# ljanyst/ssd-tensorflow

Measured on AMD Instinct MI355X. Metric: images/sec (fwd+bwd) vgg300 batch32, higher is better.
Workload: dtype f32; 1 GPU; vgg300 training step (forward + multibox loss + backward + momentum update), 32 images/GPU x 1 GPU, synthetic 300x300 BGR 0..255, GPU-encoded labels, Xavier-init weights (BASELINE.json configs[1]); global_batch=32, parallelism=dp1, allreduce=none

## Files before the change

include/ssdvgg_hip.h:

```cpp
#ifndef SSDVGG_HIP_H
#define SSDVGG_HIP_H

#include <stddef.h>

#ifdef __cplusplus
extern "C" {
#endif

typedef struct ssd_net* ssd_handle;

const char* ssd_last_error(void);
const char* ssd_version(void);

int ssd_preset_info(const char* preset, int* image_w, int* image_h, int* num_anchors, int* num_maps);
int ssd_preset_map(const char* preset, int map, int* size, double* scale, int* num_types);

int ssd_anchors(const char* preset, int device, double* out);
int ssd_anchors_abs(const char* preset, int device, int* out);

int ssd_jaccard_overlap(int device, const double* box, const double* boxes, int n, double* iou_out);

int ssd_encode_labels(const char* preset, int num_classes, int device, const double* gt_boxes,
                      const int* gt_cls, const int* gt_offsets, int b, float* vec_out);
int ssd_encode_labels_dev(const char* preset, int num_classes, int device, const double* gt_boxes,
// ... 360 lines not shown
                               int wi, int ci, int ho, int wo, int co, int kh, int kw, int stride, int dil, int pad_h, int pad_w,
                               void* stream);
int ssd_op_conv2d_dgrad_unpool_bf16(const void* dy, const void* w_io, void* dx_unpooled, const void* rec, int uh, int uw, int b,
                                    int hi, int wi, int ci, int ho, int wo, int co, int kh, int kw, int stride, int dil, int pad_h,
                                    int pad_w, void* stream);
size_t ssd_op_conv2d_dgrad_first_wgrad_bf16_ws_floats(int b, int h, int w);
int ssd_op_conv2d_dgrad_first_wgrad_bf16(const void* dy, const void* w_io, const void* mask, const float* image, float* dw1, float* dbias1,
                                         const float* w1, float weight_decay, float* ws, int b, int h, int w, void* stream);
size_t ssd_op_conv2d_wino_bits_words(int b, int hi, int wi, int ci, int ho, int wo, int co, int kh, int kw, int stride, int dil,
                                     int pad_h, int pad_w);
size_t ssd_op_conv2d_wino_ws_floats(int b, int hi, int wi, int ci, int ho, int wo, int co, int kh, int kw, int stride, int dil,
                                    int pad_h, int pad_w);
int ssd_op_conv2d_wino_fwd(const float* x, const float* w, const float* bias, float* y, float* y_pool, void* rec, void* relu_bits, float* ws,
                           int flags, int b, int hi, int wi, int ci, int ho, int wo, int co, int kh, int kw, int stride, int dil,
                           int pad_h, int pad_w, int relu, void* stream);
int ssd_op_conv2d_wino_dgrad(const float* dy, const float* w, float* dx, const float* mask, const void* mask_bits, int accumulate,
                             const void* rec, int uh, int uw, float* ws, int flags, int b, int hi, int wi, int ci, int ho, int wo, int co,
                             int kh, int kw, int stride, int dil, int pad_h, int pad_w, void* stream);
int ssd_op_conv2d_wino_wgrad(const float* x, const float* dy, float* dw, float* dbias, const float* w, float weight_decay, float* ws,
                             int flags, int b, int hi, int wi, int ci, int ho, int wo, int co, int kh, int kw, int stride, int dil,
                             int pad_h, int pad_w, void* stream);
int ssd_pool_fusion(ssd_handle h, int* out, int cap, int* count);
int ssd_debug_set_ablate(const char* tokens);

int ssd_op_clock_monitor(unsigned* out_dev, int nsamples, unsigned period_ticks, void* stream);
int ssd_op_l2norm_fwd(const float* x, const float* scale, float* y, int npix, int c, void* stream);
size_t ssd_op_l2norm_bwd_ws_floats(int npix, int c);
int ssd_op_l2norm_bwd(const float* x, const float* scale, const float* dy, float* dx, float* dscale,
                      float* ws, int npix, int c, void* stream);

// ... 12 lines not shown
```

ssd_tensorflow_amd/_lib.py:

```python
import ctypes as C
import os

_HERE = os.path.dirname(os.path.abspath(__file__))
LIB_PATH = os.environ.get('SSD_LIB') or os.path.join(_HERE, 'libssdvgg_hip.so')

if not os.path.exists(LIB_PATH):
    raise ImportError(
        f'{LIB_PATH} is missing: build it with `python -c "import __graft_entry__ as g; g.build()"` '
        f'or `make -C {os.path.join(_HERE, "csrc")}` (hipcc, gfx950). There is no CPU fallback.')

try:
    import torch
except ImportError:
    torch = None

lib = C.CDLL(LIB_PATH)

p_f32 = C.POINTER(C.c_float)
p_f64 = C.POINTER(C.c_double)
p_i32 = C.POINTER(C.c_int)
p_i64 = C.POINTER(C.c_longlong)
vp = C.c_void_p
i32 = C.c_int
f32 = C.c_float
# ... 106 lines not shown
    'ssd_merge_tiles_ws_bytes': (sz, [i32, i32]),
    'ssd_merge_tiles_dev': (i32, [vp, i32, i32, i32, vp, vp, vp, vp, vp, i32, i32, i32, vp, vp, vp, vp, vp, vp, vp, vp]),
    'ssd_merge_tiles': (i32, [i32, vp, i32, i32, i32, vp, vp, vp, vp, vp, i32, i32, i32, vp, vp, vp, vp, vp, vp]),
    'ssd_set_overlap': (i32, [handle, i32]),
    'ssd_profile_enable': (i32, [handle, i32]),
    'ssd_profile_report': (i32, [handle, C.c_char_p, sz]),
    'ssd_activation_shape': (i32, [handle, cstr, p_i32, p_i32, p_i32]),
    'ssd_activation': (i32, [handle, cstr, i32, vp, sz]),
    'ssd_op_conv2d_fwd': (i32, [vp, vp, vp, vp] + [i32] * 14 + [vp]),
    'ssd_op_conv2d_dgrad': (i32, [vp, vp, vp, vp, i32] + [i32] * 13 + [vp]),
    'ssd_op_conv2d_wgrad_ws_floats': (sz, [i32] * 13),
    'ssd_op_conv2d_wgrad': (i32, [vp, vp, vp, vp, vp, f32, vp] + [i32] * 13 + [vp]),
    'ssd_op_conv2d_wino_ws_floats': (sz, [i32] * 13),
    'ssd_op_conv2d_wino_bits_words': (sz, [i32] * 13),
    'ssd_op_conv2d_wino_fwd': (i32, [vp, vp, vp, vp, vp, vp, vp, vp, i32] + [i32] * 14 + [vp]),
    'ssd_op_conv2d_wino_dgrad': (i32, [vp, vp, vp, vp, vp, i32, vp, i32, i32, vp, i32] + [i32] * 13 + [vp]),
    'ssd_op_conv2d_wino_wgrad': (i32, [vp, vp, vp, vp, vp, f32, vp, i32] + [i32] * 13 + [vp]),
    'ssd_op_cast_filter': (i32, [vp, vp, vp, i32, i32, i32, vp]),
    'ssd_op_conv2d_fwd_bf16': (i32, [vp, vp, vp, vp, i32] + [i32] * 14 + [vp]),
    'ssd_op_conv2d_dgrad_bf16': (i32, [vp, vp, vp, vp, i32] + [i32] * 13 + [vp]),
    'ssd_op_conv2d_fwd_bf16_chain': (i32, [vp, vp, vp, vp, i32] + [i32] * 14 + [vp]),
    'ssd_op_conv2d_dgrad_bf16_chain': (i32, [vp, vp, vp, vp, i32] + [i32] * 13 + [vp]),
    'ssd_op_conv2d_wgrad_bf16_direct': (i32, [vp, vp, vp, vp, vp, f32] + [i32] * 13 + [vp]),
    'ssd_op_conv2d_wgrad_bf16_ws_floats': (sz, [i32] * 13),
    'ssd_op_conv2d_wgrad_bf16': (i32, [vp, vp, vp, vp, vp, f32, vp] + [i32] * 13 + [vp]),
    'ssd_op_conv2d_first_fwd_bf16': (i32, [vp, vp, vp, vp] + [i32] * 14 + [vp]),
    'ssd_op_conv2d_first_wgrad_bf16_ws_floats': (sz, [i32] * 13),
    'ssd_op_conv2d_first_wgrad_bf16': (i32, [vp, vp, vp, vp, vp, f32, vp] + [i32] * 13 + [vp]),
    'ssd_op_maxpool_rec_fwd': (i32, [vp, vp, vp, i32, i32, i32, i32, i32, vp]),
    'ssd_op_maxpool_rec_bwd': (i32, [vp, vp, vp, i32, i32, i32, i32, i32, i32, vp]),
# ... 74 lines not shown
```

ssd_tensorflow_amd/csrc/api.hip:

```cpp
#include "../../include/ssdvgg_hip.h"
#include "net.h"
#include "augment.h"
#include "annotate.h"
#include "jpeg.h"
#include "jpeg_enc.h"
#include "jpeg_huff.h"
#include "jpeg_huffdec.h"
#include "metrics.h"
#include <vector>
#include <map>
#include <memory>
#include <mutex>
#include <algorithm>

namespace ssd {
static thread_local std::string g_err;
void set_error(const char* fmt, ...) {
    char buf[1024];
    va_list ap;
    va_start(ap, fmt);
    vsnprintf(buf, sizeof buf, fmt, ap);
    va_end(ap);
    g_err = buf;
}
// ... 1253 lines not shown
int ssd_op_conv2d_wino_fwd(const float* x, const float* w, const float* bias, float* y, float* y_pool, void* rec, void* relu_bits, float* ws,
                           int flags, int b, int hi, int wi, int ci, int ho, int wo, int co, int kh, int kw, int stride, int dil,
                           int pad_h, int pad_w, int relu, void* stream) {
    API_BEGIN
    const ConvDesc d = mk(b, hi, wi, ci, ho, wo, co, kh, kw, stride, dil, pad_h, pad_w);
    SSD_REQUIRE(wino_applicable(d), "winograd: 3x3 / stride 1 / SAME layers (any dilation), Ci in multiples of 32, Co of 4");
    const WinoWs k(d, ws);
    if (!(flags & 1)) {
        HIP_OK(hipMemsetAsync(k.Uf, 0, (size_t)36 * d.Ci * wino_kpad(d.Co) * sizeof(float), (hipStream_t)stream));
        wino_filter(d, w, k.U, k.Uf, (hipStream_t)stream);
    }
    wino_fwd(d, x, k.U, bias, y, relu != 0, k.V, (size_t)wino_tiles(d) * d.Ci, k.Mx, y_pool, rec, (hipStream_t)stream, relu_bits,
             (flags & 4) != 0, (flags & 8) != 0);
    API_END
}
int ssd_op_conv2d_wino_dgrad(const float* dy, const float* w, float* dx, const float* mask, const void* mask_bits, int accumulate,
                             const void* rec, int uh, int uw, float* ws, int flags, int b, int hi, int wi, int ci, int ho, int wo, int co,
                             int kh, int kw, int stride, int dil, int pad_h, int pad_w, void* stream) {
    API_BEGIN
    const ConvDesc d = mk(b, hi, wi, ci, ho, wo, co, kh, kw, stride, dil, pad_h, pad_w);
    SSD_REQUIRE(wino_applicable(d), "winograd: 3x3 / stride 1 / SAME layers (any dilation), Ci in multiples of 32, Co of 4");
    const WinoWs k(d, ws);
    if (!(flags & 1)) {
        HIP_OK(hipMemsetAsync(k.Uf, 0, (size_t)36 * d.Ci * wino_kpad(d.Co) * sizeof(float), (hipStream_t)stream));
        wino_filter(d, w, k.U, k.Uf, (hipStream_t)stream);
    }
    wino_bwd_transform(d, dy, k.Yt, nullptr, (hipStream_t)stream, (flags & 8) != 0);
    wino_dgrad(d, k.Yt, k.Uf, dx, mask, accumulate != 0, k.Mx, rec, uh, uw, (hipStream_t)stream, mask_bits, (flags & 4) != 0);
    API_END
}
// ... 296 lines not shown
```

ssd_tensorflow_amd/csrc/conv.h:

```cpp
#pragma once
#include <vector>
#include "common.h"

namespace ssd {

struct ConvDesc {
    int B, Hi, Wi, Ci;
    int Ho, Wo, Co;
    int KH, KW, stride, dil;
    int pad_h, pad_w;
};

void conv_fwd(const ConvDesc& d, const float* x, const float* w, const float* bias,
              float* y, bool relu, hipStream_t s);

void conv_dgrad(const ConvDesc& d, const float* dy, const float* w, float* dx,
                const float* mask, bool accumulate, hipStream_t s);

size_t conv_wgrad_ws_floats(const ConvDesc& d);
void conv_wgrad(const ConvDesc& d, const float* x, const float* dy, float* dw, float* dbias,
                const float* w, float weight_decay, float* ws, hipStream_t s);

bool conv_fwd_pool_supported(const ConvDesc& d);
void conv_fwd_pool(const ConvDesc& d, const float* x, const float* w, const float* bias, float* y_pool, void* rec, hipStream_t s);
// ... 16 lines not shown
    static constexpr int MAX = 24;
    struct Item {
        const float* w;
        float *U, *Uf;
        int Ci, Co, Cop, blk0;
    } it[MAX];
    int n = 0, blocks = 0;
    double elems = 0;
    void add(const float* w, float* U, float* Uf, int Ci, int Co);
};
void wino_filter_plan(const WinoFilterPlan& plan, bool forward, bool flipped, hipStream_t s);
size_t wino_fwd_ws_floats(const ConvDesc& d);
void wino_fwd(const ConvDesc& d, const float* x, const float* U, const float* bias, float* y, bool relu, float* V, size_t v_ps,
              float* Mws, float* y_pool, void* pool_rec, hipStream_t s, void* relu_bits = nullptr, bool two_launch = false,
              bool ref_geom = false);
void wino_bwd_transform(const ConvDesc& d, const float* dy, float* Yt, float* Ya, hipStream_t s, bool ref_geom = false);
size_t wino_dgrad_ws_floats(const ConvDesc& d);
void wino_dgrad(const ConvDesc& d, const float* Yt, const float* Uflip, float* dx, const float* mask, bool accumulate, float* Xws,
                const void* unpool_rec, int UH, int UW, hipStream_t s, const void* mask_bits = nullptr, bool two_launch = false);
size_t wino_wgrad_ws_floats(const ConvDesc& d);
void wino_wgrad(const ConvDesc& d, const float* V, size_t v_ps, const float* Ya, float* dw, float* dbias, const float* w,
                float weight_decay, float* ws, hipStream_t s, bool ref_geom = false);

bool conv_bigk(const ConvDesc& d);
double conv_bigk_useful_flops(const ConvDesc& d);
void conv_bigk_fwd(const ConvDesc& d, const float* x, const float* w, const float* bias, float* y, bool relu, hipStream_t s);
void conv_bigk_dgrad(const ConvDesc& d, const float* dy, const float* w, float* dx, const float* mask, bool accumulate, hipStream_t s);
void conv_bigk_wgrad(const ConvDesc& d, const float* x, const float* dy, float* dw, float* dbias, const float* w, float weight_decay,
                     hipStream_t s);

// ... 128 lines not shown
```

ssd_tensorflow_amd/csrc/net.h:

```cpp
#pragma once
#include "common.h"
#include "conv.h"
#include "ops.h"
#include "boxes.h"
#include "bf16.h"
#include <string>
#include <vector>
#include <map>

namespace ssd {

struct Tensor {
    std::string name;
    int H = 0, W = 0, C = 0;
    bool relu_out = false;
    int consumers = 0;
    int done = 0;
    int gstream = 0;
    long gseq = 0;
    hipEvent_t gev = nullptr;
    bool gev_set = false;
    bool data_f32 = true;
    bool grad_f32 = true;
    void* data = nullptr;
// ... 20 lines not shown
    size_t w_off = 0, b_off = 0;
    size_t ws_off = 0;
    int k = 2;
    void* pool_rec = nullptr;
    bool fused_fwd = false, fused_bwd = false;
    int pool_after = -1, unpool = -1;
    int head = -1;
    bool fp8 = false;
    size_t sw_off = 0;
    size_t w6_off = 0;
    bool wino_f = false, wino_d = false, wino_w = false;
    float *wino_U = nullptr, *wino_Uf = nullptr, *wino_V = nullptr;
    void* wino_bits = nullptr;
    long long wino_bits_step = -1;
    long long wino_v_step = -1;
};

struct Variable {
    std::string name;
    int ndim;
    int shape[4];
    size_t off, rows, width, pitch;
    size_t count() const { return rows * width; }
};

struct DetectSlot {
    char* dev = nullptr;
    char* host = nullptr;
    size_t bytes = 0, used = 0;
    int b = 0, out_cap = 0;
// ... 185 lines not shown
```

ssd_tensorflow_amd/csrc/net.hip:

```cpp
#include "net.h"
#include <cmath>
#include <algorithm>
#include <cstdlib>
#include <atomic>
#include <mutex>

namespace ssd {

static bool first_layer_kernel(const ConvDesc& d) { return d.Ci * d.KH * d.KW <= 32 && d.Co == 64; }

int Net::add_tensor(const std::string& name, int H, int W, int C, bool relu_out) {
    Tensor t;
    t.name = name; t.H = H; t.W = W; t.C = C; t.relu_out = relu_out;
    tensors_.push_back(t);
    return (int)tensors_.size() - 1;
}

enum PadMode { PAD_SAME, PAD_VALID, PAD_BR1_VALID };

void Net::build_graph() {
    const Preset& p = *preset_;
    const int nv = C_ + 5;
    input_t_ = add_tensor("image_input", p.image_h, p.image_w, 3, false);
    int cur = input_t_;
// ... 452 lines not shown
        if (op.wino_d) {
            op.wino_Uf = (float*)hip_.mem(uf * sizeof(float));
            HIP_OK(hipMemset(op.wino_Uf, 0, uf * sizeof(float)));
            yt_max = std::max(yt_max, t * wino_kpad(d.Co));
            xw_max = std::max(xw_max, t * d.Ci);
        }
        if (op.wino_w) {
            yt_max = std::max(yt_max, t * wino_kpad(d.Co));
            for (int b = 1; b <= Bmax_; ++b) slab_max = std::max(slab_max, wino_wgrad_ws_floats(conv_desc(op, b)));
        }
        (wino_plan_first_.n == 0 && op.wino_f ? wino_plan_first_ : wino_plan_).add(params_ + op.w_off, op.wino_U, nullptr, d.Ci, d.Co);
        if (op.wino_Uf) wino_plan_flip_.add(params_ + op.w_off, nullptr, op.wino_Uf, d.Ci, d.Co);
        wino_any_f_ |= op.wino_f;
        wino_any_d_ |= op.wino_d;
    }
    if (wino_plan_.n + wino_plan_first_.n + wino_plan_flip_.n == 0) return;
    ev_wino_ = hip_.event();
    ev_wino_first_ = hip_.event();
    ev_wino_flip_ = hip_.event();
    if (m_max) for (int l = 0; l < 3; ++l) wino_m_[l] = (float*)hip_.mem(m_max * sizeof(float));
    if (v_max) for (int l = 0; l < 3; ++l) wino_vs_[l] = (float*)hip_.mem(v_max * sizeof(float));
    if (training_) {
        wino_yt_ = (float*)hip_.mem(yt_max * sizeof(float));
        wino_xw_ = (float*)hip_.mem(xw_max * sizeof(float));
        wino_ya_ = (float*)hip_.mem(yt_max * sizeof(float));
        wino_slab_ = (float*)hip_.mem(slab_max * sizeof(float));
    }
}

void Net::plan_fp8() {
// ... 403 lines not shown
        bool armed = false;
        bool done = false;
        explicit LossSlotGuard(long long& s) : seq(s) {}
        void failed() { if (armed && !done) { --seq; armed = false; } }
        ~LossSlotGuard() { if (armed && !done) --seq; }
    } fwd_guard(loss_seq_);
    if (train_mode) {
        begin_loss_slot();
        fwd_guard.armed = true;
        prof_.layer = "loss";
        l2_partials(params_, nfilters_, lw_, side ? hstream_ : stream_);
        if (nl == 2) HIP_OK(hipEventRecord(ev_l2_, hstream_));
    }
    int nl_cur = nl;
    int small_heads = 0;
    for (const int op_index : fwd_order_) {
        const Op& op = ops_[op_index];
        const Tensor& in = tensors_[op.in];
        const Tensor& out = tensors_[op.out];
        prof_.layer = op.name.c_str();
        if (op_ablated(op.name, op.kind, op.head, op.k)) continue;
        if (chain_fwd_ && in_chain_[op_index]) {
            if (op_index == chain_first_)
                for (int li = 0; li < nl_cur; ++li) {
                    Lane& ln = lane[li];
                    if (ln.cast_pending) {
                        HIP_OK(hipStreamWaitEvent(ln.s, ev_cast_, 0));
                        ln.cast_pending = false;
                    }
                    launch_tail_forward(ln.b0, ln.nb, ln.s);
                }
            continue;
        }
        if (nl_cur == 2 && heads_full && op_index == tail_first_) {
            HIP_OK(hipEventRecord(ev_join_, s2_));
            HIP_OK(hipStreamWaitEvent(stream_, ev_join_, 0));
            lane[0].nb = b;
            nl_cur = 1;
        }
        for (int li = 0; li < nl_cur; ++li) {
            Lane& ln = lane[li];
            const int nb = ln.nb;
            switch (op.kind) {
            case OP_CONV: {
                hipStream_t cs = ln.s;
                int run_nb = nb, run_b0 = ln.b0;
                if (op.head >= 0 && side) {
                    if (!ln.fmap_carried[op.head]) HIP_OK(hipEventRecord(ln.ev_fmap[op.head], ln.s));
                    ln.fmap_carried[op.head] = false;
                    if (heads_full) {
                        if (li < nl_cur - 1) break;
                        cs = (nl_cur == 1 && op.head >= 2 && (small_heads++ & 1)) ? s2_ : hstream_;
                        for (int l = 0; l < nl_cur; ++l) HIP_OK(hipStreamWaitEvent(cs, lane[l].ev_fmap[op.head], 0));
                        run_nb = b; run_b0 = 0;
                        lane[0].heads_on_side = true;
                    } else {
                        HIP_OK(hipStreamWaitEvent(ln.h, ln.ev_fmap[op.head], 0));
                        cs = ln.h;
                        ln.heads_on_side = true;
// ... 22 lines not shown
                    }
                    const size_t tpi = (size_t)wino_tiles(d) / d.B;
                    if (op.wino_V) {
                        wino_V = op.wino_V + (size_t)run_b0 * tpi * d.Ci;
                        wino_vps = (size_t)b * tpi * d.Ci;
                        if (train_mode) ops_[op_index].wino_v_step = fwd_serial_;
                    } else {
                        wino_V = wino_vs_[cs == ln.s ? li : 2];
                        wino_vps = (size_t)run_nb * tpi * d.Ci;
                    }
                    if (train_mode && op.wino_bits) {
                        wino_bits = static_cast<char*>(op.wino_bits) + (size_t)run_b0 * tpi * (d.Ci / 4) * 8;
                        ops_[op_index].wino_bits_step = fwd_serial_;
                    }
                }
                if (op.pool_after >= 0) {
                    const Op& pl = ops_[op.pool_after];
                    const Tensor& pt = tensors_[pl.out];
                    void* rec = (pl.pool_rec && train_mode)
                                    ? static_cast<char*>(pl.pool_rec) + (size_t)run_b0 * pt.H * pt.W * (pt.C / 4) * sizeof(unsigned short) : nullptr;
                    if (wino)
                        wino_fwd(d, xin, op.wino_U, params_ + op.b_off, nullptr, true, wino_V, wino_vps, wino_M,
                                 reinterpret_cast<float*>(at(pt, run_b0)), rec, cs, wino_bits);
                    else if (!bf16_)
                        conv_fwd_pool(d, xin, params_ + op.w_off, params_ + op.b_off, reinterpret_cast<float*>(at(pt, run_b0)), rec, cs);
                    else
                        conv_fwd_pool_bf16(d, reinterpret_cast<const bf16_t*>(xin), wq_oi_ + op.w_off, params_ + op.b_off,
                                           reinterpret_cast<bf16_t*>(at(pt, run_b0)), rec, cs);
                    if (run8 && pt.data8)
                        quantize8(pt, at(pt, run_b0), run_b0, run_nb, cs);
                    break;
                }
                const int fh = (side && op.head < 0 && cs == ln.s) ? head_of(op.out) : -1;
                if (fh >= 0) g_stop_event = ln.ev_fmap[fh];
                struct CarryScope {
                    bool* flag;
                    ~CarryScope() { if (flag) *flag = g_stop_event == nullptr; g_stop_event = nullptr; }
                } carry_scope{fh >= 0 ? &ln.fmap_carried[fh] : nullptr};
                if (wino)
                    wino_fwd(d, xin, op.wino_U, params_ + op.b_off, static_cast<float*>(yout), op.relu, wino_V, wino_vps, wino_M,
                             nullptr, nullptr, cs, wino_bits);
                else if (!bf16_)
                    conv_fwd(d, xin, params_ + op.w_off, params_ + op.b_off, static_cast<float*>(yout), op.relu, cs);
                else if (in.data_f32 && first_layer_kernel(d))
                    conv_first_fwd_bf16(d, xin, params_ + op.w_off, params_ + op.b_off, static_cast<bf16_t*>(yout), op.relu, cs);
                else if (in.data_f32)
                    conv_fwd_smallc_bf16out(d, xin, params_ + op.w_off, params_ + op.b_off, static_cast<bf16_t*>(yout), op.relu, cs);
                else if (run8 && op.fp8 && mx6_)
                    conv_fwd_mxfp6(d, in.data8 + (size_t)run_b0 * (in.per_image() / 32 * 24), in.scale8 + (size_t)run_b0 * (in.per_image() / 32),
                                   w8_ + op.w6_off, wsc6_ + op.sw_off, params_ + op.b_off, yout,
                                   out.data8 ? out.data8 + (size_t)run_b0 * (out.per_image() / 32 * 24) : nullptr,
                                   out.data8 ? out.scale8 + (size_t)run_b0 * (out.per_image() / 32) : nullptr,
                                   out.data8 ? (out.wants16 ? FP8_OUT_BF16_MX : FP8_OUT_MX) : FP8_OUT_BF16, op.relu, cs);
                else if (run8 && op.fp8 && mx_)
// ... 94 lines not shown
}

void Net::launch_wgrad(int op_index, int b, hipStream_t ws) {
    const Op& op = ops_[op_index];
    const Tensor& in = tensors_[op.in];
    const Tensor& out = tensors_[op.out];
    const ConvDesc d = conv_desc(op, b);
    float* slab = wgrad_ws_ + op.ws_off;
    prof_.layer = op.name.c_str();
    if (op.wino_w && op.wino_v_step == fwd_serial_) {
        const size_t tpi = (size_t)wino_tiles(d) / d.B;
        wino_bwd_transform(d, out.gf(), nullptr, wino_ya_, ws);
        wino_wgrad(d, op.wino_V, (size_t)b * tpi * d.Ci, wino_ya_, grads_ + op.w_off, grads_ + op.b_off, params_ + op.w_off, wd_,
                   wino_slab_, ws);
    } else if (!bf16_) {
        conv_wgrad(d, in.f(), out.gf(), grads_ + op.w_off, grads_ + op.b_off, params_ + op.w_off, wd_, slab, ws);
    } else if (in.data_f32) {
        if (first_layer_kernel(d))
            conv_first_wgrad_bf16(d, in.f(), out.gh(), grads_ + op.w_off, grads_ + op.b_off, params_ + op.w_off, wd_, slab, ws);
        else
            conv_wgrad_smallc_bf16dy(d, in.f(), out.gh(), grads_ + op.w_off, grads_ + op.b_off, params_ + op.w_off, wd_, slab, ws);
    } else {
        conv_wgrad_bf16(d, in.h(), out.gh(), grads_ + op.w_off, grads_ + op.b_off, params_ + op.w_off, wd_, slab, ws);
    }
}

void Net::backward_begin(int b, const float* y) {
    SSD_REQUIRE(training_, "handle was created with training = 0");
    g_prof = &prof_;
    prof_.layer = "loss";
// ... 80 lines not shown
                        if (ops_[j].kind == OP_CONV && ops_[j].out == op.in && ops_[j].in == input_t_) first = j;
                if (first >= 0 && cls == 0 && conv_dgrad_first_wgrad_bf16_applicable(d, conv_desc(ops_[first], b))) {
                    const Op& f = ops_[first];
                    prof_.layer = "conv1_2+conv1_1";
                    conv_dgrad_first_wgrad_bf16(d, out.gh(), wq_io_ + op.w_off, in.h(), conv_desc(f, b), tensors_[input_t_].f(),
                                                grads_ + f.w_off, grads_ + f.b_off, params_ + f.w_off, wd_, wgrad_ws_ + f.ws_off, ds);
                    bw_first_fused_ = true;
                    fused_first_out_ = op.in;
                    bw_wrote(cls, in);
                    bw_conv_done_[op_index] = 1;
                    lo = bw_final_lo();
                    break;
                }
                g_stop_event = dst.gev;
                struct Disarm { ~Disarm() { g_stop_event = nullptr; } } disarm;
                if (op.wino_d && cls == 0) {
                    wino_bwd_transform(d, out.gf(), wino_yt_, nullptr, ds);
                    wino_dgrad(d, wino_yt_, op.wino_Uf, up ? dst.gf() : in.gf(), mask ? in.f() : nullptr, !up && in.done > 0, wino_xw_,
                               up ? up->pool_rec : nullptr, dst.H, dst.W, ds,
                               op.wino_bits && op.wino_bits_step == fwd_serial_ ? op.wino_bits : nullptr);
                } else if (!bf16_) {
                    if (up) conv_dgrad_unpool(d, out.gf(), params_ + op.w_off, dst.gf(), up->pool_rec, dst.H, dst.W, ds);
                    else conv_dgrad(d, out.gf(), params_ + op.w_off, in.gf(), mask ? in.f() : nullptr, in.done > 0, ds);
                } else {
                    if (up) conv_dgrad_unpool_bf16(d, out.gh(), wq_io_ + op.w_off, dst.gh(), up->pool_rec, dst.H, dst.W, ds);
                    else conv_dgrad_bf16(d, out.gh(), wq_io_ + op.w_off, in.gh(), mask ? in.h() : nullptr, in.done > 0, ds);
                }
                const bool carried = dst.gev && g_stop_event == nullptr;
                bw_wrote(cls, dst, carried);
            }
            bw_conv_done_[op_index] = 1;
            lo = bw_final_lo();
            break;
        }
        case OP_POOL: {
// ... 219 lines not shown
    const bool want_bf16 = name && !strncmp(name, "bf16:", 5);
    if (want_bf16) name += 5;
    const bool want_scale = name && !want_grad && !want_bf16 && !strncmp(name, "scale:", 6);
    if (want_scale) name += 6;
    for (size_t ti = 0; ti < tensors_.size(); ++ti) {
        const Tensor& t = tensors_[ti];
        if (t.name != name || !t.data) continue;
        SSD_REQUIRE(!want_grad || t.grad != nullptr, "no gradient storage (training = 0?)");
        SSD_REQUIRE(!(want_grad && bw_first_fused_ && fused_first_out_ == (int)ti),
                    "gradient of %s is not materialised: the first layer's weight gradient was computed inside the next layer's data gradient (SSD_POOL_FUSE=3 keeps it)", name);
        for (const Op& op : ops_) {
            SSD_REQUIRE(!(op.kind == OP_POOL && op.fused_fwd && op.in == (int)ti && !want_grad),
                        "activation %s is not materialised: its 2x2 pool is fused into the convolution (SSD_POOL_FUSE=0 keeps it)", name);
            SSD_REQUIRE(!(op.kind == OP_POOL && op.fused_bwd && op.out == (int)ti && want_grad),
                        "gradient of %s is not materialised: the pool's backward is fused into its consumer's data gradient (SSD_POOL_FUSE=0 keeps it)", name);
        }
        if (want_scale) {
            SSD_REQUIRE(t.scale8 != nullptr, "activation %s has no block scales (not an MX tensor of an mxfp8 handle)", name);
            SSD_REQUIRE(count == t.per_image() / 32 * b, "scale:%s holds %zu floats for b=%d, got %zu", name, t.per_image() / 32 * b, b, count);
            HIP_OK(hipStreamSynchronize(stream_));
            std::vector<unsigned char> hs(count);
            HIP_OK(hipMemcpy(hs.data(), t.scale8, count, hipMemcpyDeviceToHost));
            for (size_t i = 0; i < count; ++i) out[i] = ldexpf(1.f, (int)hs[i] - 127);
            return;
        }
        SSD_REQUIRE(count == t.per_image() * b, "activation %s holds %zu floats for b=%d, got %zu", name, t.per_image() * b, b,
                    count);
        const void* src = want_grad ? t.grad : t.data;
        HIP_OK(hipStreamSynchronize(stream_));
        if (t.data8 && !want_grad && !want_bf16 && mx6_) {
// ... 124 lines not shown
```

ssd_tensorflow_amd/csrc/winograd.hip:

```cpp
#include "conv.h"
#include "conv_detail.h"
#include "bf16.h"
#include <algorithm>
#include <cmath>

namespace ssd {

#define LDS_PTR(p) ((__attribute__((address_space(3))) void*)(p))
constexpr unsigned WOOB = 0xFFFFFFF0u;

__device__ __forceinline__ void bt6(f32x4& d0, f32x4& d1, f32x4& d2, f32x4& d3, f32x4& d4, f32x4& d5) {
    const f32x4 t0 = 1.265625f * d0 - 2.8125f * d2 + d4;
    const f32x4 e = d4 - 2.25f * d2, f = 1.6875f * d1 - 0.75f * d3;
    const f32x4 g = d4 - 0.5625f * d2, h = 0.84375f * d1 - 1.5f * d3;
    const f32x4 t5 = 1.265625f * d1 - 2.8125f * d3 + d5;
    d0 = t0; d1 = e - f; d2 = e + f; d3 = g - h; d4 = g + h; d5 = t5;
}
__device__ __forceinline__ void a6(const f32x4 e0, const f32x4 e1, const f32x4 e2, const f32x4 e3, f32x4* u) {
    const f32x4 p = e0 + 0.5625f * e2, q = 0.75f * e1 + 0.421875f * e3;
    const f32x4 r = e0 + 2.25f * e2, t = 1.5f * e1 + 3.375f * e3;
    u[0] = e0;
    u[1] = p + q;
    u[2] = p - q;
    u[3] = r + t;
    u[4] = r - t;
    u[5] = e3;
}
template <class V>
__device__ __forceinline__ void at4(const V m0, const V m1, const V m2, const V m3, const V m4, const V m5, V* y) {
    const V s12 = m1 + m2, d12 = m1 - m2, s34 = m3 + m4, d34 = m3 - m4;
    y[0] = m0 + s12 + s34;
    y[1] = 0.75f * d12 + 1.5f * d34;
    y[2] = 0.5625f * s12 + 2.25f * s34;
    y[3] = 0.421875f * d12 + 3.375f * d34 + m5;
}

__host__ __device__ inline int bias_axis_slot(int k) { return k == 0 ? 0 : k == 1 ? 1 : k == 2 ? 2 : k == 5 ? 3 : -1; }
__device__ __forceinline__ float bias_axis_weight(int slot) {
    return slot == 0 ? -7.f / 9.f : slot == 1 ? 14.f / 9.f : slot == 2 ? 2.f / 9.f : 7.f / 16.f;
}

template <bool BT, bool AT>
__global__ __launch_bounds__(256) void wino_in_kernel(const float* __restrict__ x, float* __restrict__ V, float* __restrict__ Va,
                                                      int H, int W, int C, int Cp, int th, int tw, int T, unsigned x_bytes,
                                                      size_t v_ps, size_t va_ps, int D, unsigned long long* __restrict__ bits,
                                                      bool raster) {
    const int c4n = Cp >> 2;
    const int wg = (BT && !raster) ? xcd_remap(blockIdx.x, gridDim.x) : (int)blockIdx.x;
    const int idx = wg * 256 + threadIdx.x;
    const int q = idx % c4n, t = idx / c4n;
    if (t >= T) return;
    const int j = t % tw, t2 = t / tw;
    const int i = t2 % th, b = t2 / th;
    const int hb = (i % D) + D * 4 * (i / D), wb = (j % D) + D * 4 * (j / D);
// ... 1 lines not shown
    constexpr int LO = BT ? 0 : 1, HI = BT ? 6 : 5;
    f32x4 d[6][6];
#pragma unroll
    for (int r = LO; r < HI; ++r) {
        const int h = hb + D * (r - 1);
        const bool hv = (unsigned)h < (unsigned)H;
#pragma unroll
        for (int s = LO; s < HI; ++s) {
            const int w = wb + D * (s - 1);
            const bool ok = hv && (unsigned)w < (unsigned)W && q * 4 < C;
            const unsigned off = ok ? (unsigned)(((b * H + h) * W + w) * C + q * 4) * 4u : WOOB;
            d[r][s] = __builtin_bit_cast(f32x4, __builtin_amdgcn_raw_buffer_load_b128(rs, off, 0, 0));
        }
    }
    const size_t row = (size_t)t * Cp + q * 4;
    if constexpr (BT) {
        if (bits) {
            unsigned long long m = 0;
#pragma unroll
            for (int r = 0; r < 4; ++r)
#pragma unroll
                for (int s = 0; s < 4; ++s)
#pragma unroll
                    for (int e = 0; e < 4; ++e) m |= (unsigned long long)(d[r + 1][s + 1][e] > 0.f) << ((r * 4 + s) * 4 + e);
            bits[(size_t)t * c4n + q] = m;
        }
    }
    if constexpr (AT) {
        f32x4 c[6][4];
#pragma unroll
        for (int s = 0; s < 4; ++s) {
            f32x4 u[6];
            a6(d[1][s + 1], d[2][s + 1], d[3][s + 1], d[4][s + 1], u);
#pragma unroll
            for (int k = 0; k < 6; ++k) c[k][s] = u[k];
        }
#pragma unroll
        for (int k = 0; k < 6; ++k) {
            f32x4 u[6];
            a6(c[k][0], c[k][1], c[k][2], c[k][3], u);
#pragma unroll
            for (int l = 0; l < 6; ++l) *reinterpret_cast<f32x4*>(Va + (size_t)(k * 6 + l) * va_ps + row) = u[l];
        }
    }
    if constexpr (BT) {
#pragma unroll
        for (int s = 0; s < 6; ++s) bt6(d[0][s], d[1][s], d[2][s], d[3][s], d[4][s], d[5][s]);
#pragma unroll
        for (int r = 0; r < 6; ++r) {
            bt6(d[r][0], d[r][1], d[r][2], d[r][3], d[r][4], d[r][5]);
#pragma unroll
            for (int s = 0; s < 6; ++s) *reinterpret_cast<f32x4*>(V + (size_t)(r * 6 + s) * v_ps + row) = d[r][s];
        }
    }
}

struct WinoOutArgs {
    const float* M;
    size_t m_ps;
    float* y;
    const float* bias;
    const float* mask;
    const unsigned long long* mask_bits;
    int relu, accum;
    int H, W, N, th, tw, T;
    int D;
    unsigned short* pool_rec;
    int PH, PW;
// ... 790 lines not shown
        auto kern = wino_gemm_out_kernel<MODE, 1>;
        static bool once = (set_lds(kern, lds), true);
        (void)once;
        SSD_LAUNCH_STOP(kern, dim3(cdiv(a.M, 32) * a.NT), dim3(512), lds, s, a);
    } else {
        auto kern = wino_gemm_out_kernel<MODE, 2>;
        static bool once = (set_lds(kern, lds), true);
        (void)once;
        SSD_LAUNCH_STOP(kern, dim3(cdiv(a.M, 32) * a.NT), dim3(512), lds, s, a);
    }
    HIP_OK(hipGetLastError());
}

size_t wino_fwd_ws_floats(const ConvDesc& d) { return (size_t)36 * wino_tiles(d) * d.Co; }

void wino_fwd(const ConvDesc& d, const float* x, const float* U, const float* bias, float* y, bool relu, float* V, size_t v_ps,
              float* Mws, float* y_pool, void* pool_rec, hipStream_t s, void* relu_bits, bool two_launch, bool ref_geom) {
    require(d);
    const int T = wino_tiles(d);
    launch_in(x, V, nullptr, d.B, d.Hi, d.Wi, d.Ci, d.Ci, d.dil, v_ps, 0, s, static_cast<unsigned long long*>(relu_bits), ref_geometry(ref_geom, GEOM_IN));
    const bool fused = fuse_out(d, d.Co, d.Ci, two_launch);
    if (!fused) gemm_nn(V, v_ps, U, Mws, (size_t)T * d.Co, T, d.Co, d.Ci, s);
    WinoOutArgs a{};
    a.M = Mws; a.m_ps = (size_t)T * d.Co; a.bias = bias; a.relu = relu; a.H = d.Ho; a.W = d.Wo; a.N = d.Co;
    a.th = tiles_1d(d.Ho, d.dil); a.tw = tiles_1d(d.Wo, d.dil); a.T = T; a.D = d.dil;
    const double mb = 4.0 * 36 * T * d.Co;
    if (y_pool) {
        SSD_REQUIRE(d.dil == 1, "winograd: the fused pool is for undilated layers");
        a.y = y_pool; a.pool_rec = static_cast<unsigned short*>(pool_rec); a.PH = (d.Ho + 1) / 2; a.PW = (d.Wo + 1) / 2;
        const double ob = 4.0 * d.B * a.PH * a.PW * d.Co;
        if (fused) launch_fused<2>(V, v_ps, U, d.Ci, a, ob, s);
        else launch_out<2>(a, "wino_out_pool", mb + ob, s);
    } else {
        a.y = y;
        const double ob = 4.0 * d.B * d.Ho * d.Wo * d.Co;
// ... 108 lines not shown
```

Baseline: 1437 images/s.

## Fuse first VGG conv into the Winograd input transform of conv1_2

Adds a kernel that computes the first 3x3 conv (3 image channels to 64) with MFMA on a tile of image pixels, applies bias and ReLU, keeps the result in LDS, and writes the Winograd input transform and ReLU mask bits for the second conv directly. The first layer's 64-channel activation at full 300x300 resolution is then never written to or read back from global memory. In exchange, the halo pixels around each tile are recomputed. The weight gradient of the first layer and any activation query must now cope with that tensor being absent, so guards and a recompute path for activation queries are added.

Result: no change. 1447 images/s, median of 5 (+0.8%).

```diff
diff --git a/include/ssdvgg_hip.h b/include/ssdvgg_hip.h
--- a/include/ssdvgg_hip.h
+++ b/include/ssdvgg_hip.h
@@ -398,6 +398,9 @@
 int ssd_op_conv2d_wino_fwd(const float* x, const float* w, const float* bias, float* y, float* y_pool, void* rec, void* relu_bits, float* ws,
                            int flags, int b, int hi, int wi, int ci, int ho, int wo, int co, int kh, int kw, int stride, int dil,
                            int pad_h, int pad_w, int relu, void* stream);
+int ssd_op_conv2d_wino_fwd_first(const float* image, int image_c, const float* w1, const float* bias1, const float* w, const float* bias,
+                                 float* y, float* y_pool, void* rec, void* relu_bits, float* ws, int flags, int b, int hi, int wi, int ci,
+                                 int ho, int wo, int co, int kh, int kw, int stride, int dil, int pad_h, int pad_w, int relu, void* stream);
 int ssd_op_conv2d_wino_dgrad(const float* dy, const float* w, float* dx, const float* mask, const void* mask_bits, int accumulate,
                              const void* rec, int uh, int uw, float* ws, int flags, int b, int hi, int wi, int ci, int ho, int wo, int co,
                              int kh, int kw, int stride, int dil, int pad_h, int pad_w, void* stream);
diff --git a/ssd_tensorflow_amd/_lib.py b/ssd_tensorflow_amd/_lib.py
--- a/ssd_tensorflow_amd/_lib.py
+++ b/ssd_tensorflow_amd/_lib.py
@@ -144,6 +144,7 @@
     'ssd_op_conv2d_wino_ws_floats': (sz, [i32] * 13),
     'ssd_op_conv2d_wino_bits_words': (sz, [i32] * 13),
     'ssd_op_conv2d_wino_fwd': (i32, [vp, vp, vp, vp, vp, vp, vp, vp, i32] + [i32] * 14 + [vp]),
+    'ssd_op_conv2d_wino_fwd_first': (i32, [vp, i32, vp, vp, vp, vp, vp, vp, vp, vp, vp, i32] + [i32] * 14 + [vp]),
     'ssd_op_conv2d_wino_dgrad': (i32, [vp, vp, vp, vp, vp, i32, vp, i32, i32, vp, i32] + [i32] * 13 + [vp]),
     'ssd_op_conv2d_wino_wgrad': (i32, [vp, vp, vp, vp, vp, f32, vp, i32] + [i32] * 13 + [vp]),
     'ssd_op_cast_filter': (i32, [vp, vp, vp, i32, i32, i32, vp]),
diff --git a/ssd_tensorflow_amd/csrc/api.hip b/ssd_tensorflow_amd/csrc/api.hip
--- a/ssd_tensorflow_amd/csrc/api.hip
+++ b/ssd_tensorflow_amd/csrc/api.hip
@@ -1291,6 +1291,23 @@
              (flags & 4) != 0, (flags & 8) != 0);
     API_END
 }
+int ssd_op_conv2d_wino_fwd_first(const float* image, int image_c, const float* w1, const float* bias1, const float* w, const float* bias,
+                                 float* y, float* y_pool, void* rec, void* relu_bits, float* ws, int flags, int b, int hi, int wi, int ci,
+                                 int ho, int wo, int co, int kh, int kw, int stride, int dil, int pad_h, int pad_w, int relu, void* stream) {
+    API_BEGIN
+    const ConvDesc d = mk(b, hi, wi, ci, ho, wo, co, kh, kw, stride, dil, pad_h, pad_w);
+    const ConvDesc d1 = mk(b, hi, wi, image_c, hi, wi, ci, 3, 3, 1, 1, 1, 1);
+    SSD_REQUIRE(wino_fwd_first_applicable(d1, d),
+                "winograd, first-layer form: image channels * 9 <= 32 into 64 channels, then an undilated 3x3 / stride 1 / SAME layer");
+    const WinoWs k(d, ws);
+    if (!(flags & 1)) {
+        HIP_OK(hipMemsetAsync(k.Uf, 0, (size_t)36 * d.Ci * wino_kpad(d.Co) * sizeof(float), (hipStream_t)stream));
+        wino_filter(d, w, k.U, k.Uf, (hipStream_t)stream);
+    }
+    wino_fwd_first(d1, image, w1, bias1, d, k.U, bias, y, relu != 0, k.V, (size_t)wino_tiles(d) * d.Ci, k.Mx, y_pool, rec,
+                   (hipStream_t)stream, relu_bits, (flags & 4) != 0);
+    API_END
+}
 int ssd_op_conv2d_wino_dgrad(const float* dy, const float* w, float* dx, const float* mask, const void* mask_bits, int accumulate,
                              const void* rec, int uh, int uw, float* ws, int flags, int b, int hi, int wi, int ci, int ho, int wo, int co,
                              int kh, int kw, int stride, int dil, int pad_h, int pad_w, void* stream) {
diff --git a/ssd_tensorflow_amd/csrc/conv.h b/ssd_tensorflow_amd/csrc/conv.h
--- a/ssd_tensorflow_amd/csrc/conv.h
+++ b/ssd_tensorflow_amd/csrc/conv.h
@@ -54,6 +54,10 @@
 void wino_fwd(const ConvDesc& d, const float* x, const float* U, const float* bias, float* y, bool relu, float* V, size_t v_ps,
               float* Mws, float* y_pool, void* pool_rec, hipStream_t s, void* relu_bits = nullptr, bool two_launch = false,
               bool ref_geom = false);
+bool wino_fwd_first_applicable(const ConvDesc& d1, const ConvDesc& d);
+void wino_fwd_first(const ConvDesc& d1, const float* image, const float* w1, const float* bias1, const ConvDesc& d, const float* U,
+                    const float* bias, float* y, bool relu, float* V, size_t v_ps, float* Mws, float* y_pool, void* pool_rec, hipStream_t s,
+                    void* relu_bits = nullptr, bool two_launch = false);
 void wino_bwd_transform(const ConvDesc& d, const float* dy, float* Yt, float* Ya, hipStream_t s, bool ref_geom = false);
 size_t wino_dgrad_ws_floats(const ConvDesc& d);
 void wino_dgrad(const ConvDesc& d, const float* Yt, const float* Uflip, float* dx, const float* mask, bool accumulate, float* Xws,
diff --git a/ssd_tensorflow_amd/csrc/net.h b/ssd_tensorflow_amd/csrc/net.h
--- a/ssd_tensorflow_amd/csrc/net.h
+++ b/ssd_tensorflow_amd/csrc/net.h
@@ -58,6 +58,8 @@
     void* wino_bits = nullptr;
     long long wino_bits_step = -1;
     long long wino_v_step = -1;
+    int wino_first_into = -1, wino_first = -1;
+    long long wino_first_step = -1;
 };
 
 struct Variable {
diff --git a/ssd_tensorflow_amd/csrc/net.hip b/ssd_tensorflow_amd/csrc/net.hip
--- a/ssd_tensorflow_amd/csrc/net.hip
+++ b/ssd_tensorflow_amd/csrc/net.hip
@@ -490,6 +490,22 @@
         wino_any_f_ |= op.wino_f;
         wino_any_d_ |= op.wino_d;
     }
+    static const int first_on = env_i("SSD_WINO_FIRST", 1);
+    if (first_on)
+        for (int i = 0; i < (int)ops_.size(); ++i) {
+            Op& f = ops_[i];
+            if (f.kind != OP_CONV || f.in != input_t_ || !f.relu || f.head >= 0 || tensors_[f.out].consumers != 1) continue;
+            for (int j = 0; j < (int)ops_.size(); ++j) {
+                Op& c = ops_[j];
+                if (c.in != f.out) continue;
+                if (c.kind != OP_CONV || !c.wino_f || c.dil != 1 || c.head >= 0) break;
+                if (training_ && !(c.wino_d && c.wino_w && c.wino_bits)) break;
+                if (!wino_fwd_first_applicable(conv_desc(f, Bmax_), conv_desc(c, Bmax_))) break;
+                f.wino_first_into = j;
+                c.wino_first = i;
+                break;
+            }
+        }
     if (wino_plan_.n + wino_plan_first_.n + wino_plan_flip_.n == 0) return;
     ev_wino_ = hip_.event();
     ev_wino_first_ = hip_.event();
@@ -923,6 +939,10 @@
     }
     int nl_cur = nl;
     int small_heads = 0;
+    auto first_fused = [&](int first, int second, int li) {
+        const Op &f = ops_[first], &c = ops_[second];
+        return c.wino_f && wino_m_[li] != nullptr && !op_ablated(f.name, f.kind, f.head, f.k) && !op_ablated(c.name, c.kind, c.head, c.k);
+    };
     for (const int op_index : fwd_order_) {
         const Op& op = ops_[op_index];
         const Tensor& in = tensors_[op.in];
@@ -952,6 +972,7 @@
             const int nb = ln.nb;
             switch (op.kind) {
             case OP_CONV: {
+                if (op.wino_first_into >= 0 && first_fused(op_index, op.wino_first_into, li)) break;
                 hipStream_t cs = ln.s;
                 int run_nb = nb, run_b0 = ln.b0;
                 if (op.head >= 0 && side) {
@@ -1004,12 +1025,19 @@
                         ops_[op_index].wino_bits_step = fwd_serial_;
                     }
                 }
+                const Op* first = (wino && cs == ln.s && op.wino_first >= 0 && first_fused(op.wino_first, op_index, li)) ? &ops_[op.wino_first] : nullptr;
+                const float* image = first ? reinterpret_cast<const float*>(at(tensors_[first->in], run_b0)) : nullptr;
+                if (first) ops_[op_index].wino_first_step = fwd_serial_;
                 if (op.pool_after >= 0) {
                     const Op& pl = ops_[op.pool_after];
                     const Tensor& pt = tensors_[pl.out];
                     void* rec = (pl.pool_rec && train_mode)
                                     ? static_cast<char*>(pl.pool_rec) + (size_t)run_b0 * pt.H * pt.W * (pt.C / 4) * sizeof(unsigned short) : nullptr;
-                    if (wino)
+                    if (first)
+                        wino_fwd_first(conv_desc(*first, run_nb), image, params_ + first->w_off, params_ + first->b_off, d, op.wino_U,
+                                       params_ + op.b_off, nullptr, true, wino_V, wino_vps, wino_M, reinterpret_cast<float*>(at(pt, run_b0)),
+                                       rec, cs, wino_bits);
+                    else if (wino)
                         wino_fwd(d, xin, op.wino_U, params_ + op.b_off, nullptr, true, wino_V, wino_vps, wino_M,
                                  reinterpret_cast<float*>(at(pt, run_b0)), rec, cs, wino_bits);
                     else if (!bf16_)
@@ -1027,7 +1055,11 @@
                     bool* flag;
                     ~CarryScope() { if (flag) *flag = g_stop_event == nullptr; g_stop_event = nullptr; }
                 } carry_scope{fh >= 0 ? &ln.fmap_carried[fh] : nullptr};
-                if (wino)
+                if (first)
+                    wino_fwd_first(conv_desc(*first, run_nb), image, params_ + first->w_off, params_ + first->b_off, d, op.wino_U,
+                                   params_ + op.b_off, static_cast<float*>(yout), op.relu, wino_V, wino_vps, wino_M, nullptr, nullptr, cs,
+                                   wino_bits);
+                else if (wino)
                     wino_fwd(d, xin, op.wino_U, params_ + op.b_off, static_cast<float*>(yout), op.relu, wino_V, wino_vps, wino_M,
                              nullptr, nullptr, cs, wino_bits);
                 else if (!bf16_)
@@ -1152,6 +1184,7 @@
         wino_wgrad(d, op.wino_V, (size_t)b * tpi * d.Ci, wino_ya_, grads_ + op.w_off, grads_ + op.b_off, params_ + op.w_off, wd_,
                    wino_slab_, ws);
     } else if (!bf16_) {
+        SSD_REQUIRE(op.wino_first_step != fwd_serial_, "%s: the weight gradient would read an activation the forward pass did not write", op.name.c_str());
         conv_wgrad(d, in.f(), out.gf(), grads_ + op.w_off, grads_ + op.b_off, params_ + op.w_off, wd_, slab, ws);
     } else if (in.data_f32) {
         if (first_layer_kernel(d))
@@ -1262,11 +1295,14 @@
                 }
                 g_stop_event = dst.gev;
                 struct Disarm { ~Disarm() { g_stop_event = nullptr; } } disarm;
+                const bool bits_ok = op.wino_bits && op.wino_bits_step == fwd_serial_;
+                SSD_REQUIRE(!(mask && op.wino_first_step == fwd_serial_ && !(op.wino_d && cls == 0 && bits_ok)),
+                            "%s: the data gradient's mask would read an activation the forward pass did not write", op.name.c_str());
                 if (op.wino_d && cls == 0) {
                     wino_bwd_transform(d, out.gf(), wino_yt_, nullptr, ds);
                     wino_dgrad(d, wino_yt_, op.wino_Uf, up ? dst.gf() : in.gf(), mask ? in.f() : nullptr, !up && in.done > 0, wino_xw_,
                                up ? up->pool_rec : nullptr, dst.H, dst.W, ds,
-                               op.wino_bits && op.wino_bits_step == fwd_serial_ ? op.wino_bits : nullptr);
+                               bits_ok ? op.wino_bits : nullptr);
                 } else if (!bf16_) {
                     if (up) conv_dgrad_unpool(d, out.gf(), params_ + op.w_off, dst.gf(), up->pool_rec, dst.H, dst.W, ds);
                     else conv_dgrad(d, out.gf(), params_ + op.w_off, in.gf(), mask ? in.f() : nullptr, in.done > 0, ds);
@@ -1516,6 +1552,10 @@
                         "activation %s is not materialised: its 2x2 pool is fused into the convolution (SSD_POOL_FUSE=0 keeps it)", name);
             SSD_REQUIRE(!(op.kind == OP_POOL && op.fused_bwd && op.out == (int)ti && want_grad),
                         "gradient of %s is not materialised: the pool's backward is fused into its consumer's data gradient (SSD_POOL_FUSE=0 keeps it)", name);
+            if (op.kind == OP_CONV && op.out == (int)ti && !want_grad && op.wino_first_into >= 0 &&
+                ops_[op.wino_first_into].wino_first_step == fwd_serial_ && fwd_serial_ > 0)
+                conv_fwd(conv_desc(op, b), tensors_[input_t_].f(), params_ + op.w_off, params_ + op.b_off, static_cast<float*>(t.data), op.relu,
+                         stream_);
         }
         if (want_scale) {
             SSD_REQUIRE(t.scale8 != nullptr, "activation %s has no block scales (not an MX tensor of an mxfp8 handle)", name);
diff --git a/ssd_tensorflow_amd/csrc/winograd.hip b/ssd_tensorflow_amd/csrc/winograd.hip
--- a/ssd_tensorflow_amd/csrc/winograd.hip
+++ b/ssd_tensorflow_amd/csrc/winograd.hip
@@ -38,6 +38,28 @@
 __host__ __device__ inline int bias_axis_slot(int k) { return k == 0 ? 0 : k == 1 ? 1 : k == 2 ? 2 : k == 5 ? 3 : -1; }
 __device__ __forceinline__ float bias_axis_weight(int slot) {
     return slot == 0 ? -7.f / 9.f : slot == 1 ? 14.f / 9.f : slot == 2 ? 2.f / 9.f : 7.f / 16.f;
+}
+
+__device__ __forceinline__ void wino_bt_store(f32x4 (&d)[6][6], float* __restrict__ V, size_t v_ps, size_t row,
+                                              unsigned long long* __restrict__ bits, size_t word) {
+    if (bits) {
+        unsigned long long m = 0;
+#pragma unroll
+        for (int r = 0; r < 4; ++r)
+#pragma unroll
+            for (int s = 0; s < 4; ++s)
+#pragma unroll
+                for (int e = 0; e < 4; ++e) m |= (unsigned long long)(d[r + 1][s + 1][e] > 0.f) << ((r * 4 + s) * 4 + e);
+        bits[word] = m;
+    }
+#pragma unroll
+    for (int s = 0; s < 6; ++s) bt6(d[0][s], d[1][s], d[2][s], d[3][s], d[4][s], d[5][s]);
+#pragma unroll
+    for (int r = 0; r < 6; ++r) {
+        bt6(d[r][0], d[r][1], d[r][2], d[r][3], d[r][4], d[r][5]);
+#pragma unroll
+        for (int s = 0; s < 6; ++s) *reinterpret_cast<f32x4*>(V + (size_t)(r * 6 + s) * v_ps + row) = d[r][s];
+    }
 }
 
 template <bool BT, bool AT>
@@ -69,18 +91,6 @@
         }
     }
     const size_t row = (size_t)t * Cp + q * 4;
-    if constexpr (BT) {
-        if (bits) {
-            unsigned long long m = 0;
-#pragma unroll
-            for (int r = 0; r < 4; ++r)
-#pragma unroll
-                for (int s = 0; s < 4; ++s)
-#pragma unroll
-                    for (int e = 0; e < 4; ++e) m |= (unsigned long long)(d[r + 1][s + 1][e] > 0.f) << ((r * 4 + s) * 4 + e);
-            bits[(size_t)t * c4n + q] = m;
-        }
-    }
     if constexpr (AT) {
         f32x4 c[6][4];
 #pragma unroll
@@ -98,15 +108,130 @@
             for (int l = 0; l < 6; ++l) *reinterpret_cast<f32x4*>(Va + (size_t)(k * 6 + l) * va_ps + row) = u[l];
         }
     }
-    if constexpr (BT) {
-#pragma unroll
-        for (int s = 0; s < 6; ++s) bt6(d[0][s], d[1][s], d[2][s], d[3][s], d[4][s], d[5][s]);
-#pragma unroll
-        for (int r = 0; r < 6; ++r) {
-            bt6(d[r][0], d[r][1], d[r][2], d[r][3], d[r][4], d[r][5]);
-#pragma unroll
-            for (int s = 0; s < 6; ++s) *reinterpret_cast<f32x4*>(V + (size_t)(r * 6 + s) * v_ps + row) = d[r][s];
-        }
+    if constexpr (BT) wino_bt_store(d, V, v_ps, row, bits, (size_t)t * c4n + q);
+}
+
+constexpr int FB_R = 2, FB_C = 4;
+constexpr int FB_PH = 4 * FB_R + 2, FB_PW = 4 * FB_C + 2, FB_PIX = FB_PH * FB_PW;
+constexpr int FB_ROW = 64;
+__device__ __forceinline__ int fb_slot(int px, int c) { return px * FB_ROW + ((c ^ (px & 7)) << 2); }
+constexpr int FB_THREADS = FB_R * FB_C * 16;
+constexpr int FB_KMAX = 28;
+struct WinoFirstArgs {
+    const float* x;
+    const float* w;
+    const float* bias;
+    float* V;
+    unsigned long long* bits;
+    size_t v_ps;
+    int H, W, Ci, ntaps, th, tw, bh, bw, nblk;
+    unsigned x_bytes;
+    int tap_dh[9], tap_dw[9];
+};
+
+__device__ __forceinline__ void fb_lds_barrier() {
+    asm volatile("s_waitcnt lgkmcnt(0)" ::: "memory");
+    __builtin_amdgcn_s_barrier();
+}
+
+__global__ __launch_bounds__(FB_THREADS, 2) void wino_in_first_kernel(WinoFirstArgs p) {
+    __shared__ __attribute__((aligned(16))) float act[FB_PIX * FB_ROW];
+    __shared__ __attribute__((aligned(16))) float sbias[64];
+    __shared__ float sw[FB_KMAX * 64];
+    __shared__ int ktab[2][16][2];
+    const int tid = threadIdx.x, wave = tid >> 6, lane = tid & 63;
+    const int li = lane & 31, lh = lane >> 5;
+    const int K = p.ntaps * p.Ci;
+    for (int e = tid; e < FB_KMAX * 64; e += FB_THREADS) sw[e] = e < K * 64 ? p.w[e] : 0.f;
+    if (tid < 64) sbias[tid] = p.bias ? p.bias[tid] : 0.f;
+    if (tid < 32) {
+        const int k = 2 * (tid & 15) + (tid >> 4);
+        const bool kv = k < K;
+        const int tp = kv ? k / p.Ci : 0, c = kv ? k - tp * p.Ci : 0;
+        ktab[tid >> 4][tid & 15][0] = ((p.tap_dh[tp] * p.W + p.tap_dw[tp]) * p.Ci + c) * 4;
+        ktab[tid >> 4][tid & 15][1] = kv ? (1 << tp) : 0;
+    }
+    __syncthreads();
+    const __amdgpu_buffer_rsrc_t x_rsrc = __builtin_amdgcn_make_buffer_rsrc(const_cast<float*>(p.x), 0, p.x_bytes, 0x00020000);
+    const int tl = tid >> 4, q = tid & 15;
+    const int ty = tl / FB_C, tx = tl - ty * FB_C;
+
+    constexpr int NG = (FB_PIX + 31) / 32, NW = FB_THREADS / 64, FB_GPW = NG / NW;
+    static_assert(NG % NW == 0, "every wave takes the same number of pixel groups");
+    float xb[FB_GPW][16];
+    auto gather = [&](int blk) {
+        const int bj = blk % p.bw, b2 = blk / p.bw;
+        const int bi = b2 % p.bh, b = b2 / p.bh;
+        int lhb = lh;
+        asm volatile("" : "+v"(lhb));
+#pragma unroll
+        for (int gi = 0; gi < FB_GPW; ++gi) {
+            const int px = (wave + NW * gi) * 32 + li;
+            const int ry = px / FB_PW, rx = px - ry * FB_PW;
+            const int h = 4 * FB_R * bi - 1 + ry, w = 4 * FB_C * bj - 1 + rx;
+            const bool inside = px < FB_PIX && (unsigned)h < (unsigned)p.H && (unsigned)w < (unsigned)p.W;
+            unsigned mk = 0;
+            for (int t = 0; t < p.ntaps; ++t) {
+                const int sh = h + p.tap_dh[t], sw = w + p.tap_dw[t];
+                if ((unsigned)sh < (unsigned)p.H && (unsigned)sw < (unsigned)p.W) mk |= 1u << t;
+            }
+            if (!inside) mk = 0;
+            const unsigned base = (unsigned)(((b * p.H + h) * p.W + w) * p.Ci) * 4u;
+#pragma unroll
+            for (int j = 0; j < 16; ++j) {
+                const unsigned ok = 0u - (unsigned)((mk & (unsigned)ktab[lhb][j][1]) != 0u);
+                xb[gi][j] = __builtin_bit_cast(float, __builtin_amdgcn_raw_buffer_load_b32(x_rsrc, (int)(((base + (unsigned)ktab[lhb][j][0]) & ok) | (WOOB & ~ok)), 0, 0));
+            }
+        }
+    };
+
+    for (int blk = blockIdx.x; blk < p.nblk; blk += gridDim.x) {
+        const int bj = blk % p.bw, b2 = blk / p.bw;
+        const int bi = b2 % p.bh, b = b2 / p.bh;
+        gather(blk);
+#pragma unroll
+        for (int gi = 0; gi < FB_GPW; ++gi) {
+            const int px = (wave + NW * gi) * 32 + li;
+            const bool live = px < FB_PIX;
+            const int ry = px / FB_PW, rx = px - ry * FB_PW;
+            const int h = 4 * FB_R * bi - 1 + ry, w = 4 * FB_C * bj - 1 + rx;
+            const bool inside = live && (unsigned)h < (unsigned)p.H && (unsigned)w < (unsigned)p.W;
+#pragma unroll
+            for (int nt = 0; nt < 2; ++nt) {
+                f32x16 acc;
+#pragma unroll
+                for (int r = 0; r < 16; ++r) acc[r] = 0.f;
+#pragma unroll
+                for (int j = 0; j < 16; ++j) acc = __builtin_amdgcn_mfma_f32_32x32x2f32(2 * j + 1 < FB_KMAX ? sw[(2 * j + lh) * 64 + nt * 32 + li] : 0.f, xb[gi][j], acc, 0, 0, 0);
+#pragma unroll
+                for (int c4 = 0; c4 < 4; ++c4) {
+                    const f32x4 bv = *reinterpret_cast<const f32x4*>(sbias + nt * 32 + 8 * c4 + 4 * lh);
+                    f32x4 v;
+#pragma unroll
+                    for (int e = 0; e < 4; ++e) {
+                        v[e] = acc[4 * c4 + e] + bv[e];
+                        v[e] = v[e] > 0.f ? v[e] : 0.f;
+                        if (!inside) v[e] = 0.f;
+                    }
+                    if (live) *reinterpret_cast<f32x4*>(act + fb_slot(px, nt * 8 + 2 * c4 + lh)) = v;
+                }
+            }
+        }
+        fb_lds_barrier();
+        const int i = FB_R * bi + ty, j = FB_C * bj + tx;
+        const bool mine = i < p.th && j < p.tw;
+        if (mine) {
+            f32x4 d[6][6];
+#pragma unroll
+            for (int r = 0; r < 6; ++r)
+#pragma unroll
+                for (int s = 0; s < 6; ++s) d[r][s] = *reinterpret_cast<const f32x4*>(act + fb_slot((4 * ty + r) * FB_PW + 4 * tx + s, q));
+            const size_t t = ((size_t)b * p.th + i) * p.tw + j;
+            size_t v_ps = p.v_ps;
+            asm volatile("" : "+s"(v_ps));
+            wino_bt_store(d, p.V, v_ps, t * 64 + q * 4, p.bits, t * 16 + q);
+        }
+        fb_lds_barrier();
     }
 }
 
@@ -927,11 +1052,52 @@
 
 size_t wino_fwd_ws_floats(const ConvDesc& d) { return (size_t)36 * wino_tiles(d) * d.Co; }
 
+static void fwd_gemm_out(const ConvDesc& d, const float* U, const float* bias, float* y, bool relu, float* V, size_t v_ps, float* Mws,
+                         float* y_pool, void* pool_rec, hipStream_t s, bool two_launch);
+
 void wino_fwd(const ConvDesc& d, const float* x, const float* U, const float* bias, float* y, bool relu, float* V, size_t v_ps,
               float* Mws, float* y_pool, void* pool_rec, hipStream_t s, void* relu_bits, bool two_launch, bool ref_geom) {
     require(d);
+    launch_in(x, V, nullptr, d.B, d.Hi, d.Wi, d.Ci, d.Ci, d.dil, v_ps, 0, s, static_cast<unsigned long long*>(relu_bits), ref_geometry(ref_geom, GEOM_IN));
+    fwd_gemm_out(d, U, bias, y, relu, V, v_ps, Mws, y_pool, pool_rec, s, two_launch);
+}
+
+bool wino_fwd_first_applicable(const ConvDesc& d1, const ConvDesc& d) {
+    return conv_first_fwd_f32_applicable(d1) && d1.stride == 1 && d1.KH * d1.KW <= 9 && d1.Ci * d1.KH * d1.KW < FB_KMAX && d1.Ho == d1.Hi && d1.Wo == d1.Wi &&
+           (long long)d1.B * d1.Hi * d1.Wi * d1.Ci < (1LL << 30) - 4 &&
+           wino_applicable(d) && d.dil == 1 && d.Ci == d1.Co && d.B == d1.B && d.Hi == d1.Ho && d.Wi == d1.Wo;
+}
+
+void wino_fwd_first(const ConvDesc& d1, const float* image, const float* w1, const float* bias1, const ConvDesc& d, const float* U,
+                    const float* bias, float* y, bool relu, float* V, size_t v_ps, float* Mws, float* y_pool, void* pool_rec, hipStream_t s,
+                    void* relu_bits, bool two_launch) {
+    SSD_REQUIRE(wino_fwd_first_applicable(d1, d),
+                "winograd: the first-layer form is for a stride-1 SAME layer of Ci * taps <= 32 and 64 outputs in front of an undilated Winograd layer");
+    WinoFirstArgs a{};
+    a.x = image; a.w = w1; a.bias = bias1; a.V = V; a.bits = static_cast<unsigned long long*>(relu_bits); a.v_ps = v_ps;
+    a.H = d.Hi; a.W = d.Wi; a.Ci = d1.Ci; a.ntaps = d1.KH * d1.KW;
+    a.th = tiles_1d(d.Hi, 1); a.tw = tiles_1d(d.Wi, 1); a.bh = cdiv(a.th, FB_R); a.bw = cdiv(a.tw, FB_C);
+    a.x_bytes = (unsigned)((size_t)d1.B * d1.Hi * d1.Wi * d1.Ci * 4u);
+    for (int kh = 0; kh < d1.KH; ++kh)
+        for (int kw = 0; kw < d1.KW; ++kw) {
+            a.tap_dh[kh * d1.KW + kw] = kh * d1.dil - d1.pad_h;
+            a.tap_dw[kh * d1.KW + kw] = kw * d1.dil - d1.pad_w;
+        }
+    {
+        const double pix = (double)d.B * a.bh * a.bw * FB_PIX;
+        ProfScope prof("wino_in_first", 2.0 * pix * a.ntaps * d1.Ci * d1.Co,
+                       4.0 * ((double)d1.B * d1.Hi * d1.Wi * d1.Ci + 36.0 * wino_tiles(d) * d.Ci), s);
+        static const int cap = env_int("SSD_WINO_FIRST_GRID", 256 * 3);
+        a.nblk = d.B * a.bh * a.bw;
+        hipLaunchKernelGGL(wino_in_first_kernel, dim3((unsigned)std::min(a.nblk, cap)), dim3(FB_THREADS), 0, s, a);
+        HIP_OK(hipGetLastError());
+    }
+    fwd_gemm_out(d, U, bias, y, relu, V, v_ps, Mws, y_pool, pool_rec, s, two_launch);
+}
+
+static void fwd_gemm_out(const ConvDesc& d, const float* U, const float* bias, float* y, bool relu, float* V, size_t v_ps, float* Mws,
+                         float* y_pool, void* pool_rec, hipStream_t s, bool two_launch) {
     const int T = wino_tiles(d);
-    launch_in(x, V, nullptr, d.B, d.Hi, d.Wi, d.Ci, d.Ci, d.dil, v_ps, 0, s, static_cast<unsigned long long*>(relu_bits), ref_geometry(ref_geom, GEOM_IN));
     const bool fused = fuse_out(d, d.Co, d.Ci, two_launch);
     if (!fused) gemm_nn(V, v_ps, U, Mws, (size_t)T * d.Co, T, d.Co, d.Ci, s);
     WinoOutArgs a{};
```
